# ServiceNow/PipelineRL

Hardware: NVIDIA H100
Metric: rollout_tokens_per_s (higher is better)
Workload: dtype bf16

## Files before the change

include/prl.h:

```cpp
#ifndef PRL_H_
#define PRL_H_

#include <stddef.h>
#include <stdint.h>

#ifdef __cplusplus
extern "C" {
#endif

#define PRL_OK 0
#define PRL_ERR_INVALID (-1)
#define PRL_ERR_CUDA (-2)
#define PRL_ERR_UNSUPPORTED (-3)
#define PRL_ERR_NONFINITE (-4)

typedef void* prl_stream_t;

const char* prl_last_error(void);
int prl_version(void);
uint64_t prl_launch_count(void);
int prl_set_pdl(int32_t on);
int prl_attn_set_fused_combine(int32_t on);


enum { PRL_LOSS_PPO = 0, PRL_LOSS_REINFORCE = 1, PRL_LOSS_GSPO = 2 };

enum {
  PRL_STAT_LOSS = 0, PRL_STAT_MAX_LOSS, PRL_STAT_MIN_LOSS,
  PRL_STAT_REWARD, PRL_STAT_MAX_REWARD, PRL_STAT_MIN_REWARD,
  PRL_STAT_ENTROPY, PRL_STAT_OLD_LOGPROBS, PRL_STAT_NEW_LOGPROBS, PRL_STAT_REF_LOGPROBS,
  PRL_STAT_ADVANTAGE, PRL_STAT_MAX_ADVANTAGE, PRL_STAT_MIN_ADVANTAGE,
  PRL_STAT_KL, PRL_STAT_KL_NEW_OLD, PRL_STAT_MEAN_ABS_LOG_RATIO_NEW_OLD,
  PRL_STAT_MAX_KL, PRL_STAT_MIN_KL,
  PRL_STAT_RATIO_NEW_OLD, PRL_STAT_RATIO_NEW_OLD_SUM, PRL_STAT_RATIO_NEW_OLD_SQUARED_SUM,
  PRL_STAT_RATIO_REF_NEW, PRL_STAT_RATIO_REF_OLD,
  PRL_STAT_CLAMP_LOG_RATIO_REF_NEW_INDICATOR, PRL_STAT_CLAMP_LOG_RATIO_NEW_OLD_INDICATOR,
  PRL_STAT_TOKEN_WEIGHT, PRL_STAT_MAX_TOKEN_WEIGHT, PRL_STAT_MIN_TOKEN_WEIGHT,
  PRL_STAT_KL_COEF, PRL_STAT_ENTROPY_BONUS_COEF,
  PRL_STAT_NUM_OUTPUT_TOKENS_SUM, PRL_STAT_INPUT_SIZE,
  PRL_NUM_STATS
};

typedef struct {
  int32_t policy_loss;
  int32_t use_advantages;
  int32_t relu_log_p_weights;
  int32_t group_normalization;
  int32_t overlong_filtering;
  int32_t use_entropy_loss;
  float epsilon_low, epsilon_high;
  float clamp_log_ratio_ref_new_value;
  float kl_coef;
  float entropy_bonus_coef;
  float batch_size;
} prl_pg_config;

typedef struct {
  int64_t T;
  const float* new_logprobs;
  const float* entropy;
  const int64_t* labels;
  const float* rewards;
  const float* advantages;
  const float* ref_logprobs;
  const float* old_logprobs;
  const float* group_tokens;
  const float* num_labels;
  const float* overflow;
  const int64_t* segment_ids;
  const int64_t* position_ids;
  int32_t n_segments;
  int32_t num_sequences;
  int32_t sentinel;
} prl_pg_batch;

size_t prl_pg_workspace_bytes(int32_t max_segments);

int prl_pg_loss_fwd_bwd(const prl_pg_batch* batch, const prl_pg_config* cfg,
                        float* loss, float* dloss_dlogprob, float* dloss_dentropy,
                        double* stats, int32_t* nonfinite,
                        void* workspace, size_t workspace_bytes, prl_stream_t stream);

int prl_pg_gspo_segment_sums(const prl_pg_batch* batch, const prl_pg_config* cfg, double* seg_sums, prl_stream_t stream);
int prl_pg_loss_fwd_bwd_seg(const prl_pg_batch* batch, const prl_pg_config* cfg, float* loss, float* dloss_dlogprob,
                            float* dloss_dentropy, double* stats, int32_t* nonfinite, void* workspace,
                            size_t workspace_bytes, const double* seg_sums, const double* seg_local_count,
                            prl_stream_t stream);

int prl_logprob_tail_fwd(const float* logits, int64_t T, int64_t V, int64_t row_stride,
                         const int64_t* input_ids, float temperature,
                         float* new_logprobs , float* entropy ,
                         float* lse , prl_stream_t stream);
int prl_logprob_tail_bwd(const float* logits, int64_t T, int64_t V, int64_t row_stride,
                         const int64_t* input_ids, float temperature,
                         const float* lse, const float* entropy,
                         const float* g_logprobs, const float* g_entropy,
                         float* dlogits, int64_t dlogits_stride, prl_stream_t stream);

int prl_logprob_rows_bwd(const float* logits, int64_t n_rows, int64_t V, int64_t row_stride,
                         const int64_t* targets , float temperature, const float* lse,
                         const float* entropy, const float* g_logprobs, const float* g_entropy,
                         float* dlogits, int64_t dlogits_stride, prl_stream_t stream);
int prl_head_dlogits(const void* W_bf16, const void* W_lo_bf16, const void* X_bf16, int64_t M, int64_t V, int64_t K,
                     float temperature, const int64_t* targets, const float* lse, const float* entropy,
                     const float* g_logprobs, const float* g_entropy, void* dz_bf16, int64_t ld_dz, prl_stream_t stream);
// ... 273 lines not shown
```

pipelinerl_b200/_lib.py:

```python
from __future__ import annotations

import ctypes as C
from pathlib import Path

_LIB_PATH = Path(__file__).resolve().parent / "_lib" / "libprl.so"
_lib = None


class PrlError(RuntimeError):
    def __init__(self, code: int, msg: str):
        super().__init__(f"libprl error {code}: {msg}")
        self.code = code


class NonFiniteError(AssertionError):
    """Mirrors the reference's `assert torch.isfinite(...)` (rl/__init__.py:213,263,291,386)."""


class PgConfig(C.Structure):
    _fields_ = [
        ("policy_loss", C.c_int32), ("use_advantages", C.c_int32), ("relu_log_p_weights", C.c_int32),
        ("group_normalization", C.c_int32), ("overlong_filtering", C.c_int32), ("use_entropy_loss", C.c_int32),
        ("epsilon_low", C.c_float), ("epsilon_high", C.c_float), ("clamp_log_ratio_ref_new_value", C.c_float),
        ("kl_coef", C.c_float), ("entropy_bonus_coef", C.c_float), ("batch_size", C.c_float),
# ... 10 lines not shown
        ("n_segments", C.c_int32), ("num_sequences", C.c_int32), ("sentinel", C.c_int32),
    ]


class AdamwArgs(C.Structure):
    _fields_ = [
        ("n", C.c_int64),
        ("master", C.c_void_p), ("exp_avg", C.c_void_p), ("exp_avg_sq", C.c_void_p),
        ("grad", C.c_void_p), ("grad_is_bf16", C.c_int32),
        ("param_bf16", C.c_void_p), ("param_bf16_lo", C.c_void_p),
        ("tensor_offsets", C.c_void_p), ("tensor_no_decay", C.c_void_p), ("n_tensors", C.c_int32),
        ("lr", C.c_double), ("beta1", C.c_double), ("beta2", C.c_double), ("eps", C.c_double),
        ("weight_decay", C.c_double), ("step", C.c_int32), ("max_grad_norm", C.c_float),
        ("grad_scale", C.c_float),
    ]


class AdamwShardArgs(C.Structure):
    _fields_ = [
        ("n", C.c_int64), ("shard_begin", C.c_int64), ("shard_end", C.c_int64),
        ("master", C.c_void_p), ("exp_avg", C.c_void_p), ("exp_avg_sq", C.c_void_p),
        ("grads", C.c_void_p * 8), ("shadows", C.c_void_p * 8), ("norm_tables", C.c_void_p * 8),
        ("n_peers", C.c_int32), ("rank", C.c_int32), ("grad_is_bf16", C.c_int32),
        ("gsum_scratch", C.c_void_p), ("tensor_offsets", C.c_void_p), ("tensor_no_decay", C.c_void_p),
        ("n_tensors", C.c_int32),
        ("lr", C.c_double), ("beta1", C.c_double), ("beta2", C.c_double), ("eps", C.c_double), ("weight_decay", C.c_double),
        ("step", C.c_int32), ("max_grad_norm", C.c_float), ("grad_scale", C.c_float),
    ]


class EngineState(C.Structure):
    _fields_ = [
        ("B", C.c_int32), ("sampled", C.c_void_p), ("sampled_logprobs", C.c_void_p), ("tokens", C.c_void_p),
        ("positions", C.c_void_p), ("seq_lens", C.c_void_p), ("active", C.c_void_p), ("prompt_buf", C.c_void_p),
        ("prompt_stride", C.c_int32), ("prompt_len", C.c_void_p), ("out_ids", C.c_void_p),
        ("out_logprobs", C.c_void_p), ("out_stride", C.c_int32), ("gen_count", C.c_void_p), ("max_new", C.c_void_p),
        ("finished", C.c_void_p), ("eos_id", C.c_int32), ("ignore_eos", C.c_int32), ("ignore_eos_rows", C.c_void_p),
        ("stop_ids", C.c_void_p), ("stop_stride", C.c_int32), ("n_stop", C.c_void_p), ("stop_reason", C.c_void_p),
    ]


class StopStrings(C.Structure):
    _fields_ = [
        ("tok_bytes", C.c_void_p), ("tok_offsets", C.c_void_p), ("tok_special", C.c_void_p), ("vocab", C.c_int32),
        ("stop_str", C.c_void_p), ("stop_str_fail", C.c_void_p), ("stop_str_len", C.c_void_p), ("n_stop_str", C.c_void_p),
        ("max_stop_str", C.c_int32), ("stop_str_stride", C.c_int32), ("stop_str_flags", C.c_void_p),
        ("stop_str_state", C.c_void_p), ("stop_str_match", C.c_void_p), ("min_tokens", C.c_void_p),
    ]


class MbRecord(C.Structure):
    _fields_ = [("n_chunk", C.c_int32), ("n_pack", C.c_int32), ("padding", C.c_int32), ("total_tok", C.c_int32),
                ("total_lp", C.c_int32), ("n_stat_slots", C.c_int32), ("n_rollout_slots", C.c_int32), ("n_groups", C.c_int32),
                ("reward", C.c_void_p), ("stat_slot", C.c_void_p), ("rollout_slot", C.c_void_p), ("group_slot", C.c_void_p),
                ("n_tok_all", C.c_void_p), ("pack_idx", C.c_void_p), ("pack_flags", C.c_void_p), ("tok_off", C.c_void_p),
                ("lp_off", C.c_void_p), ("input_ids", C.c_void_p), ("labels", C.c_void_p), ("logprobs", C.c_void_p),
                ("ref_logprobs", C.c_void_p)]


class MbColumns(C.Structure):
    _fields_ = [(k, C.c_void_p) for k in ("input_ids", "labels", "attention_mask", "position_ids", "segment_ids", "rewards",
                                          "advantages", "ref_logprobs", "old_logprobs", "group_tokens", "num_labels",
                                          "overflow", "seq_boundaries")]


PRL_NUM_STATS = 32
LOSS_IDS = {"ppo": 0, "reinforce": 1, "gspo": 2}
STAT_NAMES = [
    "loss", "max_loss", "min_loss", "reward", "max_reward", "min_reward", "entropy", "old_logprobs",
    "new_logprobs", "ref_logprobs", "advantage", "max_advantage", "min_advantage", "kl", "kl_new_old",
    "mean_abs_log_ratio_new_old", "max_kl", "min_kl", "ratio_new_old", "ratio_new_old_sum",
    "ratio_new_old_squared_sum", "ratio_ref_new", "ratio_ref_old", "clamp_log_ratio_ref_new_indicator",
    "clamp_log_ratio_new_old_indicator", "token_weight", "max_token_weight", "min_token_weight", "kl_coef",
    "entropy_bonus_coef", "num_output_tokens_sum", "input_size",
]
assert len(STAT_NAMES) == PRL_NUM_STATS

_SIGNATURES = {
    "prl_last_error": (C.c_char_p, []),
    "prl_version": (C.c_int, []),
    "prl_launch_count": (C.c_uint64, []),
    "prl_set_pdl": (C.c_int, [C.c_int32]),
    "prl_attn_set_fused_combine": (C.c_int, [C.c_int32]),
    "prl_pg_workspace_bytes": (C.c_size_t, [C.c_int32]),
    "prl_pg_loss_fwd_bwd": (C.c_int, [C.POINTER(PgBatch), C.POINTER(PgConfig), C.c_void_p, C.c_void_p, C.c_void_p,
                                      C.c_void_p, C.c_void_p, C.c_void_p, C.c_size_t, C.c_void_p]),
    "prl_pg_gspo_segment_sums": (C.c_int, [C.POINTER(PgBatch), C.POINTER(PgConfig), C.c_void_p, C.c_void_p]),
    "prl_pg_loss_fwd_bwd_seg": (C.c_int, [C.POINTER(PgBatch), C.POINTER(PgConfig), C.c_void_p, C.c_void_p, C.c_void_p,
                                          C.c_void_p, C.c_void_p, C.c_void_p, C.c_size_t, C.c_void_p, C.c_void_p, C.c_void_p]),
    "prl_logprob_tail_fwd": (C.c_int, [C.c_void_p, C.c_int64, C.c_int64, C.c_int64, C.c_void_p, C.c_float,
                                       C.c_void_p, C.c_void_p, C.c_void_p, C.c_void_p]),
    "prl_logprob_tail_bwd": (C.c_int, [C.c_void_p, C.c_int64, C.c_int64, C.c_int64, C.c_void_p, C.c_float,
                                       C.c_void_p, C.c_void_p, C.c_void_p, C.c_void_p, C.c_void_p, C.c_int64,
                                       C.c_void_p]),
    "prl_gemm_auto_split_k": (C.c_int, [C.c_int64, C.c_int64, C.c_int64]),
    "prl_gemm_set_smem_budget_kb": (C.c_int, [C.c_int32]),
    "prl_gemm_set_tiled_weights": (C.c_int, [C.c_int32]),
    "prl_gemm_tn": (C.c_int, [C.c_void_p, C.c_int64, C.c_void_p, C.c_int64, C.c_int64, C.c_int64, C.c_int64,
                              C.c_void_p, C.c_int64, C.c_int32, C.c_int32, C.c_void_p, C.c_void_p, C.c_int64,
                              C.c_float, C.c_void_p]),
    "prl_rowops_workspace_bytes": (C.c_size_t, [C.c_int64]),
    "prl_rmsnorm_fwd": (C.c_int, [C.c_void_p, C.c_void_p, C.c_int64, C.c_int64, C.c_float, C.c_void_p, C.c_void_p,
                                  C.c_void_p]),
    "prl_rmsnorm_bwd": (C.c_int, [C.c_void_p, C.c_void_p, C.c_void_p, C.c_void_p, C.c_void_p, C.c_int64, C.c_int64,
                                  C.c_void_p, C.c_void_p, C.c_void_p, C.c_size_t, C.c_void_p]),
    "prl_colsum_bf16": (C.c_int, [C.c_void_p, C.c_int64, C.c_int64, C.c_int64, C.c_void_p, C.c_void_p, C.c_size_t,
                                  C.c_void_p]),
    "prl_rope_inplace": (C.c_int, [C.c_void_p, C.c_int64, C.c_int64, C.c_int32, C.c_int32, C.c_void_p, C.c_void_p,
                                   C.c_float, C.c_void_p]),
    "prl_qk_norm_rope_fwd": (C.c_int, [C.c_void_p, C.c_int64, C.c_int64, C.c_int32, C.c_int32, C.c_int32, C.c_void_p,
                                       C.c_void_p, C.c_float, C.c_void_p, C.c_void_p, C.c_void_p, C.c_void_p, C.c_void_p]),
    "prl_qk_norm_rope_bwd": (C.c_int, [C.c_void_p, C.c_int64, C.c_int64, C.c_int32, C.c_int32, C.c_int32, C.c_void_p,
                                       C.c_void_p, C.c_void_p, C.c_void_p, C.c_void_p, C.c_void_p, C.c_void_p, C.c_void_p,
                                       C.c_void_p, C.c_size_t, C.c_void_p]),
    "prl_silu_mul_fwd": (C.c_int, [C.c_void_p, C.c_int64, C.c_int64, C.c_void_p, C.c_void_p]),
    "prl_silu_mul_bwd": (C.c_int, [C.c_void_p, C.c_void_p, C.c_int64, C.c_int64, C.c_void_p, C.c_void_p]),
    "prl_embed_gather": (C.c_int, [C.c_void_p, C.c_void_p, C.c_int64, C.c_int64, C.c_void_p, C.c_void_p]),
    "prl_embed_scatter_add": (C.c_int, [C.c_void_p, C.c_void_p, C.c_void_p, C.c_int64, C.c_int64, C.c_void_p]),
    "prl_gemm_ex": (C.c_int, [C.c_void_p, C.c_int64, C.c_int32, C.c_void_p, C.c_int64, C.c_int32, C.c_int64, C.c_int64,
                              C.c_int64, C.c_void_p, C.c_int64, C.c_int32, C.c_int32, C.c_void_p, C.c_void_p, C.c_int64,
                              C.c_float, C.c_void_p]),
    "prl_transpose_bf16": (C.c_int, [C.c_void_p, C.c_int64, C.c_int64, C.c_int64, C.c_void_p, C.c_int64, C.c_void_p]),
    "prl_gemm_bf16_splitk": (C.c_int, [C.c_void_p, C.c_void_p, C.c_void_p, C.c_int64, C.c_int64, C.c_int64, C.c_int32,
                                       C.c_void_p, C.c_void_p]),
    "prl_head_workspace_bytes": (C.c_size_t, [C.c_int64, C.c_int64]),
    "prl_head_logprob": (C.c_int, [C.c_void_p, C.c_void_p, C.c_void_p, C.c_int64, C.c_int64, C.c_int64, C.c_float,
                                   C.c_void_p, C.c_int32, C.c_uint64, C.c_uint32, C.c_void_p, C.c_void_p, C.c_void_p,
                                   C.c_void_p, C.c_void_p, C.c_void_p, C.c_size_t, C.c_void_p]),
    "prl_embed_rmsnorm": (C.c_int, [C.c_void_p, C.c_void_p, C.c_void_p, C.c_float, C.c_int32, C.c_int32, C.c_int32,
                                    C.c_void_p, C.c_void_p, C.c_void_p]),
    "prl_residual_rmsnorm": (C.c_int, [C.c_void_p, C.c_int32, C.c_int32, C.c_int32, C.c_void_p, C.c_float,
                                       C.c_void_p, C.c_void_p, C.c_void_p, C.c_size_t, C.c_void_p]),
    "prl_qkv_rope_cache": (C.c_int, [C.c_void_p, C.c_int32, C.c_int32, C.c_void_p, C.c_int32, C.c_int32, C.c_int32,
                                     C.c_void_p, C.c_void_p, C.c_int32, C.c_void_p, C.c_void_p, C.c_void_p, C.c_void_p,
                                     C.c_int64, C.c_int32, C.c_int32, C.c_void_p, C.c_size_t, C.c_void_p]),
    "prl_qkv_norm_rope_cache": (C.c_int, [C.c_void_p, C.c_int32, C.c_int32, C.c_void_p, C.c_void_p, C.c_void_p, C.c_float,
                                          C.c_int32, C.c_int32, C.c_int32, C.c_void_p, C.c_void_p, C.c_int32, C.c_void_p,
                                          C.c_void_p, C.c_void_p, C.c_void_p, C.c_int64, C.c_int32, C.c_int32, C.c_void_p,
                                          C.c_size_t, C.c_void_p]),
    "prl_paged_attn_prefill_tc": (C.c_int, [C.c_void_p, C.c_int32, C.c_void_p, C.c_int64, C.c_int32, C.c_int32, C.c_void_p,
                                            C.c_int32, C.c_void_p, C.c_void_p, C.c_void_p, C.c_void_p, C.c_int32,
                                            C.c_int32, C.c_int32, C.c_int32, C.c_int32, C.c_int32, C.c_float,
                                            C.c_void_p, C.c_void_p]),
    "prl_attn_varlen_fwd": (C.c_int, [C.c_void_p, C.c_int64, C.c_int32, C.c_void_p, C.c_void_p, C.c_int32, C.c_int32,
                                      C.c_int32, C.c_int32, C.c_int32, C.c_float, C.c_void_p, C.c_void_p, C.c_void_p]),
    "prl_attn_set_fwd_generation": (C.c_int, [C.c_int32]),
    "prl_attn_set_bwd_generation": (C.c_int, [C.c_int32]),
    "prl_attn_set_prefill_generation": (C.c_int, [C.c_int32]),
    "prl_attn_varlen_bwd_workspace_bytes": (C.c_size_t, [C.c_int32, C.c_int32]),
    "prl_attn_varlen_fwd_kv": (C.c_int, [C.c_void_p, C.c_int64, C.c_int32, C.c_void_p, C.c_int64, C.c_int32, C.c_void_p,
                                         C.c_void_p, C.c_void_p, C.c_void_p, C.c_int32, C.c_int32, C.c_int32, C.c_int32,
                                         C.c_int32, C.c_float, C.c_void_p, C.c_void_p, C.c_void_p]),
    "prl_attn_varlen_bwd_kv": (C.c_int, [C.c_void_p, C.c_int64, C.c_int32, C.c_void_p, C.c_int64, C.c_int32, C.c_void_p,
                                         C.c_void_p, C.c_void_p, C.c_void_p, C.c_int32, C.c_int32, C.c_int32, C.c_int32,
                                         C.c_int32, C.c_int32, C.c_float, C.c_void_p, C.c_void_p, C.c_void_p, C.c_void_p,
                                         C.c_int64, C.c_void_p, C.c_int64, C.c_void_p, C.c_size_t, C.c_void_p]),
    "prl_attn_varlen_bwd": (C.c_int, [C.c_void_p, C.c_int64, C.c_int32, C.c_void_p, C.c_void_p, C.c_int32, C.c_int32,
                                      C.c_int32, C.c_int32, C.c_int32, C.c_float, C.c_void_p, C.c_void_p, C.c_void_p,
                                      C.c_void_p, C.c_int64, C.c_void_p, C.c_size_t, C.c_void_p]),
    "prl_paged_attn_prefill": (C.c_int, [C.c_void_p, C.c_void_p, C.c_int64, C.c_int32, C.c_int32, C.c_void_p,
                                         C.c_int32, C.c_void_p, C.c_void_p, C.c_void_p, C.c_void_p, C.c_int32,
                                         C.c_int32, C.c_int32, C.c_int32, C.c_int32, C.c_int32, C.c_float,
                                         C.c_void_p, C.c_void_p]),
    "prl_silu_mul": (C.c_int, [C.c_void_p, C.c_int32, C.c_int32, C.c_int32, C.c_void_p, C.c_void_p, C.c_size_t,
                               C.c_void_p]),
    "prl_paged_attn_splits": (C.c_int, [C.c_int32, C.c_int32, C.c_int32]),
# ... 97 lines not shown
```

pipelinerl_b200/csrc/decode_ops.cu:

```cuda
#include "prl_common.cuh"
#include <math.h>

namespace prl {
namespace {

__device__ __forceinline__ void l2_prefetch_range(const void* ptr, size_t bytes, size_t tid, size_t nthreads) {
  if (!ptr) return;
  const char* base = static_cast<const char*>(ptr);
  const size_t n_lines = bytes >> 7;
  for (size_t i = tid; i < n_lines; i += nthreads)
    asm volatile("prefetch.global.L2::evict_last [%0];" ::"l"(base + (i << 7)));
}

__device__ __forceinline__ float block_sum(float v, float* s_red) {
  v = warp_sum(v);
  const int lane = threadIdx.x & 31, warp = threadIdx.x >> 5;
  if (lane == 0) s_red[warp] = v;
  __syncthreads();
  float t = 0.f;
  const int nw = (blockDim.x + 31) >> 5;
  for (int i = 0; i < nw; ++i) t += s_red[i];
  __syncthreads();
  return t;
}

__global__ void __launch_bounds__(256) embed_rmsnorm_kernel(const int32_t* __restrict__ tokens,
                                                           const __nv_bfloat16* __restrict__ embed,
                                                           const __nv_bfloat16* __restrict__ gamma, float eps, int H,
                                                           int vocab, float* __restrict__ h,
                                                           __nv_bfloat16* __restrict__ x) {
  pdl_launch_dependents();
  pdl_wait();
  __shared__ float s_red[32];
  const int b = blockIdx.x;
  int tok = tokens[b];
  if (tok < 0 || tok >= vocab) tok = 0;
  const __nv_bfloat16* row = embed + (int64_t)tok * H;
  float ss = 0.f;
  for (int i = threadIdx.x; i < H; i += blockDim.x) {
    const float v = __bfloat162float(row[i]);
    h[(int64_t)b * H + i] = v;
    ss += v * v;
  }
  const float tot = block_sum(ss, s_red);
  const float r = rsqrtf(tot / (float)H + eps);
  for (int i = threadIdx.x; i < H; i += blockDim.x) {
    const float v = __bfloat162float(row[i]);
    x[(int64_t)b * H + i] = __float2bfloat16_rn(v * r * __bfloat162float(gamma[i]));
  }
}

constexpr int kMaxSplitUnroll = 8;
__global__ void __launch_bounds__(1024) residual_rmsnorm_kernel(const float* __restrict__ part, int n_split, int B,
                                                               int H, const __nv_bfloat16* __restrict__ gamma,
                                                               float eps, float* __restrict__ h,
                                                               __nv_bfloat16* __restrict__ x, const void* pf_ptr,
                                                               size_t pf_bytes) {
  pdl_launch_dependents();
  l2_prefetch_range(pf_ptr, pf_bytes, (size_t)blockIdx.x * blockDim.x + threadIdx.x, (size_t)gridDim.x * blockDim.x);
  pdl_wait();
  extern __shared__ float s_row[];
  __shared__ float s_red[32];
  const int b = blockIdx.x;
  const int H4 = H >> 2;
  float4* hrow = reinterpret_cast<float4*>(h + (int64_t)b * H);
  float ss = 0.f;
  float4 keep = make_float4(0.f, 0.f, 0.f, 0.f);
  const bool single = H4 <= (int)blockDim.x;
  for (int i = threadIdx.x; i < H4; i += blockDim.x) {
    float4 v = hrow[i];
    for (int s = 0; s < n_split; s += kMaxSplitUnroll) {
      float4 p[kMaxSplitUnroll];
#pragma unroll
      for (int u = 0; u < kMaxSplitUnroll; ++u)
        if (s + u < n_split) p[u] = reinterpret_cast<const float4*>(part + ((int64_t)(s + u) * B + b) * H)[i];
#pragma unroll
      for (int u = 0; u < kMaxSplitUnroll; ++u)
        if (s + u < n_split) { v.x += p[u].x; v.y += p[u].y; v.z += p[u].z; v.w += p[u].w; }
    }
    hrow[i] = v;
    if (single) keep = v; else reinterpret_cast<float4*>(s_row)[i] = v;
    ss += v.x * v.x + v.y * v.y + v.z * v.z + v.w * v.w;
  }
  const float tot = block_sum(ss, s_red);
  const float r = rsqrtf(tot / (float)H + eps);
  for (int i = threadIdx.x; i < H4; i += blockDim.x) {
    const float4 v = single ? keep : reinterpret_cast<const float4*>(s_row)[i];
    const uint2 gw = reinterpret_cast<const uint2*>(gamma)[i];
    const float g0 = bf16_bits_to_float(gw.x & 0xffffu), g1 = bf16_bits_to_float(gw.x >> 16);
    const float g2 = bf16_bits_to_float(gw.y & 0xffffu), g3 = bf16_bits_to_float(gw.y >> 16);
    const uint32_t o0 = float_to_bf16_bits(v.x * r * g0), o1 = float_to_bf16_bits(v.y * r * g1);
    const uint32_t o2 = float_to_bf16_bits(v.z * r * g2), o3 = float_to_bf16_bits(v.w * r * g3);
    reinterpret_cast<uint2*>(x + (int64_t)b * H)[i] = make_uint2(o0 | (o1 << 16), o2 | (o3 << 16));
  }
}


__device__ __forceinline__ float head_sumsq(float x1, float x2, float* s_ss) {
  float v = warp_sum(__fadd_rn(__fmul_rn(x1, x1), __fmul_rn(x2, x2)));
  const int warp = threadIdx.x >> 5;
  __syncthreads();
  if ((threadIdx.x & 31) == 0) s_ss[warp] = v;
  __syncthreads();
  const int w0 = warp & ~1;
  return __fadd_rn(s_ss[w0], s_ss[w0 + 1]);
}

__device__ __forceinline__ float head_rstd(float ss, float eps) { return rsqrtf(__fmaf_rn(ss, 1.f / 128.f, eps)); }

template <bool kNorm>
__global__ void __launch_bounds__(64) qkv_rope_cache_kernel(const float* __restrict__ part, int n_split, int B,
                                                           const __nv_bfloat16* __restrict__ bias,
                                                           const __nv_bfloat16* __restrict__ q_gamma,
                                                           const __nv_bfloat16* __restrict__ k_gamma, float eps,
                                                           int n_q, int n_kv,
// ... 575 lines not shown
```

pipelinerl_b200/csrc/paged_attn.cu:

```cuda
#include "prl_common.cuh"
#include "tc_ptx.cuh"
#include <math.h>

namespace prl {
namespace {

constexpr int kPage = 64;
constexpr int kD = 128;
constexpr int kStages = 6;
constexpr int kStageBytes = 4 * 8192;
constexpr int kConsumers = 4;
constexpr int kThreads = (kConsumers + 1) * 32;
constexpr int kMaxPagesPerSplit = 1024;

struct AttnParams {
  const __nv_bfloat16* q;
  const int32_t* block_table;
  const int32_t* seq_lens;
  int max_blocks, n_q, n_kv, R;
  int64_t n_pages;
  int layer, n_splits;
  float scale_log2;
  float* o_part;
  float* ml_part;
  unsigned int* tickets;
  __nv_bfloat16* out;
};

__device__ __forceinline__ void ldsm_x4(uint32_t addr, uint32_t& r0, uint32_t& r1, uint32_t& r2, uint32_t& r3) {
  asm volatile("ldmatrix.sync.aligned.m8n8.x4.shared.b16 {%0,%1,%2,%3}, [%4];"
               : "=r"(r0), "=r"(r1), "=r"(r2), "=r"(r3) : "r"(addr));
}
__device__ __forceinline__ void ldsm_x4_t(uint32_t addr, uint32_t& r0, uint32_t& r1, uint32_t& r2, uint32_t& r3) {
  asm volatile("ldmatrix.sync.aligned.m8n8.x4.trans.shared.b16 {%0,%1,%2,%3}, [%4];"
               : "=r"(r0), "=r"(r1), "=r"(r2), "=r"(r3) : "r"(addr));
}
__device__ __forceinline__ void mma_bf16(float (&c)[4], const uint32_t (&a)[4], uint32_t b0, uint32_t b1) {
  asm volatile(
      "mma.sync.aligned.m16n8k16.row.col.f32.bf16.bf16.f32 {%0,%1,%2,%3}, {%4,%5,%6,%7}, {%8,%9}, {%0,%1,%2,%3};"
      : "+f"(c[0]), "+f"(c[1]), "+f"(c[2]), "+f"(c[3])
      : "r"(a[0]), "r"(a[1]), "r"(a[2]), "r"(a[3]), "r"(b0), "r"(b1));
}
__device__ __forceinline__ uint32_t pack_bf16(float lo, float hi) {
  __nv_bfloat162 v = __floats2bfloat162_rn(lo, hi);
  return *reinterpret_cast<uint32_t*>(&v);
}
__device__ __forceinline__ float fast_exp2(float x) {
  float y;
  asm("ex2.approx.ftz.f32 %0, %1;" : "=f"(y) : "f"(x));
  return y;
}

__global__ void __launch_bounds__(kThreads, 1)
paged_attn_decode_kernel(const __grid_constant__ CUtensorMap tm_kv, AttnParams p) {
  extern __shared__ uint8_t smem_raw[];
  const uint32_t base = (ptx::smem_u32(smem_raw) + 1023u) & ~1023u;
  uint8_t* base_ptr = smem_raw + (base - ptx::smem_u32(smem_raw));
  const uint32_t bar_base = base + kStages * kStageBytes;
  auto full_bar = [&](int s) { return bar_base + 8u * (uint32_t)s; };
  auto empty_bar = [&](int s) { return bar_base + 8u * (uint32_t)(kStages + s); };
  int32_t* s_pages = reinterpret_cast<int32_t*>(base_ptr + kStages * kStageBytes + 8 * 2 * kStages);

  const int split = blockIdx.x, kvh = blockIdx.y, b = blockIdx.z;
  const int warp = threadIdx.x >> 5, lane = threadIdx.x & 31;
  pdl_launch_dependents();
  pdl_wait();
  const int seq_len = p.seq_lens[b];
  const int n_pages_b = (seq_len + kPage - 1) / kPage;
  const int per_split = (n_pages_b + p.n_splits - 1) / p.n_splits;
  const int p_begin = split * per_split;
  const int p_end = (p_begin + per_split < n_pages_b) ? p_begin + per_split : n_pages_b;
  const int n_it = p_end > p_begin ? p_end - p_begin : 0;
  const int R = p.R;

  auto finish = [&]() {
    if (p.tickets == nullptr) return;
    __shared__ unsigned int s_ticket;
    __threadfence();
    __syncthreads();
    if (threadIdx.x == 0) s_ticket = atomicAdd(&p.tickets[b * p.n_kv + kvh], 1u);
    __syncthreads();
    if (s_ticket != (unsigned)(p.n_splits - 1)) return;
    __threadfence();
    for (int i = threadIdx.x; i < R * kD; i += kThreads) {
      const int r = i / kD, d = i % kD;
      const int64_t head = (int64_t)b * p.n_q + kvh * R + r;
      float M = -INFINITY;
      for (int sp = 0; sp < p.n_splits; ++sp) M = fmaxf(M, __ldcg(&p.ml_part[(head * p.n_splits + sp) * 2]));
      float L = 0.f, O = 0.f;
      for (int sp = 0; sp < p.n_splits; ++sp) {
        const float ms = __ldcg(&p.ml_part[(head * p.n_splits + sp) * 2]);
        const float f = (ms == -INFINITY) ? 0.f : fast_exp2(ms - M);
        L += __ldcg(&p.ml_part[(head * p.n_splits + sp) * 2 + 1]) * f;
        O += __ldcg(&p.o_part[(head * p.n_splits + sp) * kD + d]) * f;
      }
      p.out[head * kD + d] = __float2bfloat16_rn(L > 0.f ? O / L : 0.f);
    }
    if (threadIdx.x == 0) p.tickets[b * p.n_kv + kvh] = 0u;
  };

  if (n_it == 0) {
    for (int i = threadIdx.x; i < R * kD; i += kThreads) {
      const int r = i / kD, d = i % kD;
      const int64_t head = (int64_t)b * p.n_q + kvh * R + r;
      p.o_part[(head * p.n_splits + split) * kD + d] = 0.f;
      if (d == 0) {
        p.ml_part[(head * p.n_splits + split) * 2 + 0] = -INFINITY;
        p.ml_part[(head * p.n_splits + split) * 2 + 1] = 0.f;
      }
    }
    finish();
    return;
  }

  if (threadIdx.x == 0) {
    for (int s = 0; s < kStages; ++s) {
      ptx::mbar_init(full_bar(s), 1);
      ptx::mbar_init(empty_bar(s), kConsumers);
    }
    ptx::fence_barrier_init();
    ptx::prefetch_tensormap(&tm_kv);
  }
  for (int i = threadIdx.x; i < n_it; i += kThreads)
    s_pages[i] = p.block_table[(int64_t)b * p.max_blocks + p_begin + i];
  __syncthreads();

  float m_run[2] = {-INFINITY, -INFINITY}, l_run[2] = {0.f, 0.f};
  float o[16][4];
#pragma unroll
  for (int i = 0; i < 16; ++i) { o[i][0] = o[i][1] = o[i][2] = o[i][3] = 0.f; }
  const int g = lane >> 2, t = lane & 3;

  if (warp == kConsumers) {
    if (lane == 0) {
      for (int it = 0; it < n_it; ++it) {
        const int s = it % kStages;
        const uint32_t ph = (uint32_t)((it / kStages) & 1);
        ptx::mbar_wait(empty_bar(s), ph ^ 1u);
        ptx::mbar_arrive_expect_tx(full_bar(s), kStageBytes);
        const int page = s_pages[it];
        const int row_k = (int)(((((int64_t)p.layer * 2 + 0) * p.n_pages + page) * p.n_kv + kvh) * kPage);
        const int row_v = (int)(((((int64_t)p.layer * 2 + 1) * p.n_pages + page) * p.n_kv + kvh) * kPage);
        const uint32_t dst = base + (uint32_t)(s * kStageBytes);
        ptx::tma_load_2d(dst, &tm_kv, 0, row_k, full_bar(s), ptx::kEvictFirst);
        ptx::tma_load_2d(dst + 8192, &tm_kv, 64, row_k, full_bar(s), ptx::kEvictFirst);
        ptx::tma_load_2d(dst + 16384, &tm_kv, 0, row_v, full_bar(s), ptx::kEvictFirst);
        ptx::tma_load_2d(dst + 24576, &tm_kv, 64, row_v, full_bar(s), ptx::kEvictFirst);
      }
    }
  } else {
    uint32_t qa[8][4];
    {
      const __nv_bfloat16* qb = p.q + ((int64_t)b * p.n_q + kvh * R) * kD;
#pragma unroll
      for (int ks = 0; ks < 8; ++ks) {
        const int c = ks * 16 + 2 * t;
        qa[ks][0] = (g < R) ? *reinterpret_cast<const uint32_t*>(qb + g * kD + c) : 0u;
        qa[ks][1] = (g + 8 < R) ? *reinterpret_cast<const uint32_t*>(qb + (g + 8) * kD + c) : 0u;
        qa[ks][2] = (g < R) ? *reinterpret_cast<const uint32_t*>(qb + g * kD + c + 8) : 0u;
        qa[ks][3] = (g + 8 < R) ? *reinterpret_cast<const uint32_t*>(qb + (g + 8) * kD + c + 8) : 0u;
      }
    }
    const int mi = lane >> 3, lr = lane & 7;
    for (int it = 0; it < n_it; ++it) {
      const int s = it % kStages;
      const uint32_t ph = (uint32_t)((it / kStages) & 1);
      ptx::mbar_wait(full_bar(s), ph);
      const uint32_t kbase = base + (uint32_t)(s * kStageBytes);
      const uint32_t vbase = kbase + 16384;

      float sc[2][4] = {{0.f, 0.f, 0.f, 0.f}, {0.f, 0.f, 0.f, 0.f}};
      {
        const int row = warp * 16 + (mi >> 1) * 8 + lr;
#pragma unroll
        for (int ks = 0; ks < 8; ++ks) {
          const int chunk = ks * 2 + (mi & 1);
          const uint32_t addr = kbase + (uint32_t)((chunk >> 3) * 8192 + row * 128 + (((chunk & 7) ^ (row & 7)) << 4));
          uint32_t r0, r1, r2, r3;
          ldsm_x4(addr, r0, r1, r2, r3);
          mma_bf16(sc[0], qa[ks], r0, r1);
          mma_bf16(sc[1], qa[ks], r2, r3);
        }
      }
      const int tok0 = (p_begin + it) * kPage + warp * 16;
      const bool tail = tok0 + 16 > seq_len;
#pragma unroll
      for (int nt = 0; nt < 2; ++nt)
#pragma unroll
        for (int e = 0; e < 4; ++e) {
          float v = sc[nt][e] * p.scale_log2;
          if (tail && (tok0 + nt * 8 + 2 * t + (e & 1)) >= seq_len) v = -INFINITY;
          sc[nt][e] = v;
        }
      uint32_t pa[4];
#pragma unroll
      for (int r = 0; r < 2; ++r) {
        float mx = fmaxf(fmaxf(sc[0][2 * r], sc[0][2 * r + 1]), fmaxf(sc[1][2 * r], sc[1][2 * r + 1]));
        mx = fmaxf(mx, __shfl_xor_sync(0xffffffffu, mx, 1));
        mx = fmaxf(mx, __shfl_xor_sync(0xffffffffu, mx, 2));
        const float m_new = fmaxf(m_run[r], mx);
        const float m_use = (m_new == -INFINITY) ? 0.f : m_new;
        const float alpha = fast_exp2(m_run[r] - m_use);
        const float p00 = fast_exp2(sc[0][2 * r] - m_use), p01 = fast_exp2(sc[0][2 * r + 1] - m_use);
        const float p10 = fast_exp2(sc[1][2 * r] - m_use), p11 = fast_exp2(sc[1][2 * r + 1] - m_use);
        l_run[r] = l_run[r] * alpha + (p00 + p01 + p10 + p11);
        m_run[r] = m_new;
#pragma unroll
        for (int i = 0; i < 16; ++i) { o[i][2 * r] *= alpha; o[i][2 * r + 1] *= alpha; }
        pa[r] = pack_bf16(p00, p01);
        pa[2 + r] = pack_bf16(p10, p11);
      }
      {
        const int row = warp * 16 + (mi & 1) * 8 + lr;
#pragma unroll
        for (int dn = 0; dn < 8; ++dn) {
          const int chunk = dn * 2 + (mi >> 1);
          const uint32_t addr = vbase + (uint32_t)((chunk >> 3) * 8192 + row * 128 + (((chunk & 7) ^ (row & 7)) << 4));
          uint32_t r0, r1, r2, r3;
          ldsm_x4_t(addr, r0, r1, r2, r3);
          mma_bf16(o[2 * dn], pa, r0, r1);
          mma_bf16(o[2 * dn + 1], pa, r2, r3);
        }
      }
      __syncwarp();
      if (lane == 0) ptx::mbar_arrive(empty_bar(s));
    }
#pragma unroll
    for (int r = 0; r < 2; ++r) {
      l_run[r] += __shfl_xor_sync(0xffffffffu, l_run[r], 1);
      l_run[r] += __shfl_xor_sync(0xffffffffu, l_run[r], 2);
    }
  }

// ... 167 lines not shown
          const int qpos = pos_first + g + ((e >> 1) ? 8 : 0);
          if (key > qpos) v = -INFINITY;
        }
        sc[nt][e] = v;
      }
#pragma unroll
    for (int r = 0; r < 2; ++r) {
      float mx = -INFINITY;
#pragma unroll
      for (int nt = 0; nt < 8; ++nt) mx = fmaxf(mx, fmaxf(sc[nt][2 * r], sc[nt][2 * r + 1]));
      mx = fmaxf(mx, __shfl_xor_sync(0xffffffffu, mx, 1));
      mx = fmaxf(mx, __shfl_xor_sync(0xffffffffu, mx, 2));
      const float m_new = fmaxf(m_run[r], mx);
      const float m_use = (m_new == -INFINITY) ? 0.f : m_new;
      const float alpha = fast_exp2(m_run[r] - m_use);
      float sum = 0.f;
#pragma unroll
      for (int nt = 0; nt < 8; ++nt) {
        sc[nt][2 * r] = fast_exp2(sc[nt][2 * r] - m_use);
        sc[nt][2 * r + 1] = fast_exp2(sc[nt][2 * r + 1] - m_use);
        sum += sc[nt][2 * r] + sc[nt][2 * r + 1];
      }
      l_run[r] = l_run[r] * alpha + sum;
      m_run[r] = m_new;
#pragma unroll
      for (int i = 0; i < 16; ++i) { o[i][2 * r] *= alpha; o[i][2 * r + 1] *= alpha; }
    }
#pragma unroll
    for (int j = 0; j < 4; ++j) {
      uint32_t pa[4];
      pa[0] = pack_bf16(sc[2 * j][0], sc[2 * j][1]);
      pa[1] = pack_bf16(sc[2 * j][2], sc[2 * j][3]);
      pa[2] = pack_bf16(sc[2 * j + 1][0], sc[2 * j + 1][1]);
      pa[3] = pack_bf16(sc[2 * j + 1][2], sc[2 * j + 1][3]);
      const int row = j * 16 + (mi & 1) * 8 + lr;
#pragma unroll
      for (int dn = 0; dn < 8; ++dn) {
        const int chunk = dn * 2 + (mi >> 1);
        const uint32_t addr = vbase + (uint32_t)((chunk >> 3) * 8192 + row * 128 + (((chunk & 7) ^ (row & 7)) << 4));
        uint32_t r0, r1, r2, r3;
        ldsm_x4_t(addr, r0, r1, r2, r3);
        mma_bf16(o[2 * dn], pa, r0, r1);
        mma_bf16(o[2 * dn + 1], pa, r2, r3);
      }
    }
    __syncwarp();
    if (lane == 0) ptx::mbar_arrive(empty_bar(s));
  }
#pragma unroll
  for (int r = 0; r < 2; ++r) {
    l_run[r] += __shfl_xor_sync(0xffffffffu, l_run[r], 1);
    l_run[r] += __shfl_xor_sync(0xffffffffu, l_run[r], 2);
    const int rowi = g + 8 * r;
    if (rowi < n_valid) {
      const float inv = l_run[r] > 0.f ? 1.f / l_run[r] : 0.f;
      __nv_bfloat16* dst = p.out + ((int64_t)(row0 + rowi) * p.n_q + head) * kD;
#pragma unroll
      for (int i = 0; i < 16; ++i)
        *reinterpret_cast<uint32_t*>(dst + i * 8 + 2 * t) = pack_bf16(o[i][2 * r] * inv, o[i][2 * r + 1] * inv);
    }
  }
}

__global__ void __launch_bounds__(kD) attn_combine_kernel(const float* __restrict__ o_part,
                                                         const float* __restrict__ ml_part, int n_splits,
                                                         __nv_bfloat16* __restrict__ out) {
  const int64_t head = blockIdx.x;
  const int d = threadIdx.x;
  pdl_launch_dependents();
  pdl_wait();
  float M = -INFINITY;
  for (int s = 0; s < n_splits; ++s) M = fmaxf(M, ml_part[(head * n_splits + s) * 2]);
  float L = 0.f, O = 0.f;
  for (int s = 0; s < n_splits; ++s) {
    const float ms = ml_part[(head * n_splits + s) * 2];
    const float f = (ms == -INFINITY) ? 0.f : fast_exp2(ms - M);
    L += ml_part[(head * n_splits + s) * 2 + 1] * f;
    O += o_part[(head * n_splits + s) * kD + d] * f;
  }
  out[head * kD + d] = __float2bfloat16_rn(L > 0.f ? O / L : 0.f);
}

static int g_fused_combine = 0;

}
}

using namespace prl;

extern "C" int prl_attn_set_fused_combine(int32_t on) {
  g_fused_combine = on ? 1 : 0;
  return PRL_OK;
}

extern "C" int prl_paged_attn_splits(int32_t B, int32_t n_kv, int32_t max_seq_len) {
  const int pages = (max_seq_len + kPage - 1) / kPage;
  const int sms = num_sms();
  int splits = 1;
  while (B * n_kv * splits < 2 * sms && pages / (splits * 2) >= 4) splits *= 2;
  while ((pages + splits - 1) / splits > kMaxPagesPerSplit) splits *= 2;
  return splits;
}

extern "C" size_t prl_paged_attn_workspace_bytes(int32_t B, int32_t n_q, int32_t n_splits) {
  return (size_t)B * n_q * n_splits * (kD + 2) * sizeof(float) + (size_t)B * n_q * sizeof(unsigned int);
}

extern "C" int prl_paged_attn_decode(const void* q, const void* kv_cache, int64_t n_pages, int32_t n_layers,
                                     int32_t layer, const int32_t* block_table, int32_t max_blocks,
                                     const int32_t* seq_lens, int32_t B, int32_t n_q, int32_t n_kv, int32_t head_dim,
                                     int32_t page_size, int32_t n_splits, float sm_scale, void* out_bf16,
                                     void* workspace, size_t workspace_bytes, prl_stream_t stream_) {
  PRL_CHECK_ARG(q && kv_cache && block_table && seq_lens && out_bf16 && workspace, "prl_paged_attn_decode: NULL argument");
  PRL_CHECK_ARG(head_dim == kD && page_size == kPage, "prl_paged_attn_decode: head_dim must be 128 and page_size 64");
  PRL_CHECK_ARG(B >= 1 && n_kv >= 1 && n_q % n_kv == 0 && n_q / n_kv <= 16, "prl_paged_attn_decode: need n_q/n_kv <= 16");
  PRL_CHECK_ARG(n_splits >= 1 && layer >= 0 && layer < n_layers, "prl_paged_attn_decode: bad layer/splits");
  PRL_CHECK_ARG((max_blocks + n_splits - 1) / n_splits <= kMaxPagesPerSplit,
                "prl_paged_attn_decode: %d blocks / %d splits exceeds %d pages per CTA", max_blocks, n_splits,
                kMaxPagesPerSplit);
  PRL_CHECK_ARG(workspace_bytes >= prl_paged_attn_workspace_bytes(B, n_q, n_splits), "prl_paged_attn_decode: workspace too small");
  const int64_t total_rows = (int64_t)n_layers * 2 * n_pages * n_kv * kPage;
  PRL_CHECK_ARG(total_rows < (1ll << 31), "prl_paged_attn_decode: KV cache too large for 32-bit TMA row coordinates");
  CUtensorMap tm;
  int rc = make_tmap_2d_bf16(&tm, kv_cache, kD, (uint64_t)total_rows, kD * 2, 64, kPage);
  if (rc) return rc;
  AttnParams p;
  p.q = (const __nv_bfloat16*)q;
  p.block_table = block_table;
  p.seq_lens = seq_lens;
  p.max_blocks = max_blocks; p.n_q = n_q; p.n_kv = n_kv; p.R = n_q / n_kv;
  p.n_pages = n_pages; p.layer = layer; p.n_splits = n_splits;
  p.scale_log2 = sm_scale * 1.4426950408889634f;
  p.o_part = (float*)workspace;
  p.ml_part = p.o_part + (size_t)B * n_q * n_splits * kD;
  p.tickets = g_fused_combine ? reinterpret_cast<unsigned int*>(p.ml_part + (size_t)B * n_q * n_splits * 2) : nullptr;
  p.out = (__nv_bfloat16*)out_bf16;
  const int smem = kStages * kStageBytes + 1024 + 8 * 2 * kStages + 4 * kMaxPagesPerSplit + 16;
  static SmemAttr smem_attr = {};
  PRL_CUDA(ensure_smem(paged_attn_decode_kernel, smem, smem_attr));
  cudaStream_t stream = (cudaStream_t)stream_;
  dim3 grid((unsigned)n_splits, (unsigned)n_kv, (unsigned)B);
  PRL_CUDA(launch_pdl(paged_attn_decode_kernel, grid, dim3(kThreads), (size_t)smem, stream, tm, p));
  PRL_LAUNCH_CHECK();
  if (!g_fused_combine) {
    PRL_CUDA(launch_pdl(attn_combine_kernel, dim3((unsigned)(B * n_q)), dim3(kD), 0, stream, (const float*)p.o_part,
                        (const float*)p.ml_part, (int)n_splits, (__nv_bfloat16*)out_bf16));
    PRL_LAUNCH_CHECK();
  }
  return PRL_OK;
}

extern "C" int prl_paged_attn_prefill(const void* q, const void* kv_cache, int64_t n_pages, int32_t n_layers,
                                      int32_t layer, const int32_t* block_table, int32_t max_blocks,
                                      const int32_t* seq_q_start, const int32_t* seq_q_len, const int32_t* seq_pos0,
                                      const int32_t* seq_slot, int32_t n_seqs, int32_t max_q_len, int32_t n_q,
                                      int32_t n_kv, int32_t head_dim, int32_t page_size, float sm_scale,
                                      void* out_bf16, prl_stream_t stream_) {
  PRL_CHECK_ARG(q && kv_cache && block_table && seq_q_start && seq_q_len && seq_pos0 && seq_slot && out_bf16,
                "prl_paged_attn_prefill: NULL argument");
  PRL_CHECK_ARG(head_dim == kD && page_size == kPage, "prl_paged_attn_prefill: head_dim must be 128 and page_size 64");
  PRL_CHECK_ARG(n_seqs >= 1 && max_q_len >= 1 && n_kv >= 1 && n_q % n_kv == 0 && n_q / n_kv <= kPrefillMaxR,
                "prl_paged_attn_prefill: need n_q/n_kv <= %d", kPrefillMaxR);
  PRL_CHECK_ARG(layer >= 0 && layer < n_layers, "prl_paged_attn_prefill: bad layer");
  const int64_t total_rows = (int64_t)n_layers * 2 * n_pages * n_kv * kPage;
  PRL_CHECK_ARG(total_rows < (1ll << 31), "prl_paged_attn_prefill: KV cache too large for 32-bit TMA row coordinates");
  CUtensorMap tm;
  int rc = make_tmap_2d_bf16(&tm, kv_cache, kD, (uint64_t)total_rows, kD * 2, 64, kPage);
  if (rc) return rc;
  PrefillParams p;
  p.q = (const __nv_bfloat16*)q; p.out = (__nv_bfloat16*)out_bf16;
  p.block_table = block_table; p.seq_q_start = seq_q_start; p.seq_q_len = seq_q_len; p.seq_pos0 = seq_pos0;
  p.seq_slot = seq_slot; p.max_blocks = max_blocks; p.n_q = n_q; p.n_kv = n_kv; p.R = n_q / n_kv;
  p.n_pages = n_pages; p.layer = layer; p.scale_log2 = sm_scale * 1.4426950408889634f;
  const int smem = kStages * kStageBytes + 1024 + 8 * 2 * kStages + 16;
  static SmemAttr smem_attr = {};
  PRL_CUDA(ensure_smem(paged_attn_prefill_kernel, smem, smem_attr));
  dim3 grid((unsigned)((max_q_len + 15) / 16), (unsigned)n_kv, (unsigned)n_seqs);
  PRL_CUDA(launch_pdl(paged_attn_prefill_kernel, grid, dim3((p.R + 1) * 32), (size_t)smem, (cudaStream_t)stream_, tm, p));
  PRL_LAUNCH_CHECK();
  return PRL_OK;
}
```

Measured before the change: 3786.

## Prefetch KV pages before PDL wait and stage fused combine partials in shared memory

Paged attention decode now reads seq_lens and the block table, then issues TMA loads for up to kStages KV pages that are already complete, all before griddepcontrol.wait. This overlaps KV fetch with the tail of the previous kernel. The last page is excluded because it may still be written by the upstream kernel. The fused combine path first copies the split partials into shared memory, so the merge no longer reads global memory repeatedly. The embed kernel now waits on the prior grid before signalling dependents. This relies on the earlier pages and the block table staying unchanged during the prior kernel, which would be a correctness risk if that assumption fails.

New measurement: 3790 (median of 6 runs). No clear change (+0.1%).

```diff
diff --git a/include/prl.h b/include/prl.h
--- a/include/prl.h
+++ b/include/prl.h
@@ -21,6 +21,7 @@
 uint64_t prl_launch_count(void);
 int prl_set_pdl(int32_t on);
 int prl_attn_set_fused_combine(int32_t on);
+int prl_attn_set_prewait(int32_t on);
 
 
 enum { PRL_LOSS_PPO = 0, PRL_LOSS_REINFORCE = 1, PRL_LOSS_GSPO = 2 };
diff --git a/pipelinerl_b200/_lib.py b/pipelinerl_b200/_lib.py
--- a/pipelinerl_b200/_lib.py
+++ b/pipelinerl_b200/_lib.py
@@ -116,6 +116,7 @@
     "prl_launch_count": (C.c_uint64, []),
     "prl_set_pdl": (C.c_int, [C.c_int32]),
     "prl_attn_set_fused_combine": (C.c_int, [C.c_int32]),
+    "prl_attn_set_prewait": (C.c_int, [C.c_int32]),
     "prl_pg_workspace_bytes": (C.c_size_t, [C.c_int32]),
     "prl_pg_loss_fwd_bwd": (C.c_int, [C.POINTER(PgBatch), C.POINTER(PgConfig), C.c_void_p, C.c_void_p, C.c_void_p,
                                       C.c_void_p, C.c_void_p, C.c_void_p, C.c_size_t, C.c_void_p]),
diff --git a/pipelinerl_b200/csrc/decode_ops.cu b/pipelinerl_b200/csrc/decode_ops.cu
--- a/pipelinerl_b200/csrc/decode_ops.cu
+++ b/pipelinerl_b200/csrc/decode_ops.cu
@@ -29,8 +29,8 @@
                                                            const __nv_bfloat16* __restrict__ gamma, float eps, int H,
                                                            int vocab, float* __restrict__ h,
                                                            __nv_bfloat16* __restrict__ x) {
-  pdl_launch_dependents();
-  pdl_wait();
+  pdl_wait();
+  pdl_launch_dependents();
   __shared__ float s_red[32];
   const int b = blockIdx.x;
   int tok = tokens[b];
diff --git a/pipelinerl_b200/csrc/paged_attn.cu b/pipelinerl_b200/csrc/paged_attn.cu
--- a/pipelinerl_b200/csrc/paged_attn.cu
+++ b/pipelinerl_b200/csrc/paged_attn.cu
@@ -20,6 +20,7 @@
   int max_blocks, n_q, n_kv, R;
   int64_t n_pages;
   int layer, n_splits;
+  int prewait;
   float scale_log2;
   float* o_part;
   float* ml_part;
@@ -64,8 +65,8 @@
   const int split = blockIdx.x, kvh = blockIdx.y, b = blockIdx.z;
   const int warp = threadIdx.x >> 5, lane = threadIdx.x & 31;
   pdl_launch_dependents();
-  pdl_wait();
-  const int seq_len = p.seq_lens[b];
+  if (!p.prewait) pdl_wait();
+  const int seq_len = __ldcg(&p.seq_lens[b]);
   const int n_pages_b = (seq_len + kPage - 1) / kPage;
   const int per_split = (n_pages_b + p.n_splits - 1) / p.n_splits;
   const int p_begin = split * per_split;
@@ -82,24 +83,40 @@
     __syncthreads();
     if (s_ticket != (unsigned)(p.n_splits - 1)) return;
     __threadfence();
+    const int64_t head0 = (int64_t)b * p.n_q + kvh * R;
+    const float* op = p.o_part + head0 * p.n_splits * kD;
+    const float* ml = p.ml_part + head0 * p.n_splits * 2;
+    const int n_o = R * p.n_splits * kD, n_ml = R * p.n_splits * 2;
+    const bool staged = (n_o + n_ml) * (int)sizeof(float) <= kStages * kStageBytes;
+    if (staged) {
+      float* s_part = reinterpret_cast<float*>(base_ptr);
+#pragma unroll 4
+      for (int i = threadIdx.x; i < n_o / 4; i += kThreads)
+        reinterpret_cast<float4*>(s_part)[i] = __ldcg(reinterpret_cast<const float4*>(op) + i);
+      for (int i = threadIdx.x; i < n_ml; i += kThreads) s_part[n_o + i] = __ldcg(ml + i);
+      __syncthreads();
+      op = s_part;
+      ml = s_part + n_o;
+    }
+    auto ld = [&](const float* a) { return staged ? *a : __ldcg(a); };
     for (int i = threadIdx.x; i < R * kD; i += kThreads) {
       const int r = i / kD, d = i % kD;
-      const int64_t head = (int64_t)b * p.n_q + kvh * R + r;
       float M = -INFINITY;
-      for (int sp = 0; sp < p.n_splits; ++sp) M = fmaxf(M, __ldcg(&p.ml_part[(head * p.n_splits + sp) * 2]));
+      for (int sp = 0; sp < p.n_splits; ++sp) M = fmaxf(M, ld(&ml[(r * p.n_splits + sp) * 2]));
       float L = 0.f, O = 0.f;
       for (int sp = 0; sp < p.n_splits; ++sp) {
-        const float ms = __ldcg(&p.ml_part[(head * p.n_splits + sp) * 2]);
+        const float ms = ld(&ml[(r * p.n_splits + sp) * 2]);
         const float f = (ms == -INFINITY) ? 0.f : fast_exp2(ms - M);
-        L += __ldcg(&p.ml_part[(head * p.n_splits + sp) * 2 + 1]) * f;
-        O += __ldcg(&p.o_part[(head * p.n_splits + sp) * kD + d]) * f;
-      }
-      p.out[head * kD + d] = __float2bfloat16_rn(L > 0.f ? O / L : 0.f);
+        L += ld(&ml[(r * p.n_splits + sp) * 2 + 1]) * f;
+        O += ld(&op[(r * p.n_splits + sp) * kD + d]) * f;
+      }
+      p.out[(head0 + r) * kD + d] = __float2bfloat16_rn(L > 0.f ? O / L : 0.f);
     }
     if (threadIdx.x == 0) p.tickets[b * p.n_kv + kvh] = 0u;
   };
 
   if (n_it == 0) {
+    pdl_wait();
     for (int i = threadIdx.x; i < R * kD; i += kThreads) {
       const int r = i / kD, d = i % kD;
       const int64_t head = (int64_t)b * p.n_q + kvh * R + r;
@@ -122,7 +139,7 @@
     ptx::prefetch_tensormap(&tm_kv);
   }
   for (int i = threadIdx.x; i < n_it; i += kThreads)
-    s_pages[i] = p.block_table[(int64_t)b * p.max_blocks + p_begin + i];
+    s_pages[i] = __ldcg(&p.block_table[(int64_t)b * p.max_blocks + p_begin + i]);
   __syncthreads();
 
   float m_run[2] = {-INFINITY, -INFINITY}, l_run[2] = {0.f, 0.f};
@@ -132,23 +149,32 @@
   const int g = lane >> 2, t = lane & 3;
 
   if (warp == kConsumers) {
-    if (lane == 0) {
-      for (int it = 0; it < n_it; ++it) {
-        const int s = it % kStages;
-        const uint32_t ph = (uint32_t)((it / kStages) & 1);
-        ptx::mbar_wait(empty_bar(s), ph ^ 1u);
-        ptx::mbar_arrive_expect_tx(full_bar(s), kStageBytes);
-        const int page = s_pages[it];
-        const int row_k = (int)(((((int64_t)p.layer * 2 + 0) * p.n_pages + page) * p.n_kv + kvh) * kPage);
-        const int row_v = (int)(((((int64_t)p.layer * 2 + 1) * p.n_pages + page) * p.n_kv + kvh) * kPage);
-        const uint32_t dst = base + (uint32_t)(s * kStageBytes);
-        ptx::tma_load_2d(dst, &tm_kv, 0, row_k, full_bar(s), ptx::kEvictFirst);
-        ptx::tma_load_2d(dst + 8192, &tm_kv, 64, row_k, full_bar(s), ptx::kEvictFirst);
-        ptx::tma_load_2d(dst + 16384, &tm_kv, 0, row_v, full_bar(s), ptx::kEvictFirst);
-        ptx::tma_load_2d(dst + 24576, &tm_kv, 64, row_v, full_bar(s), ptx::kEvictFirst);
-      }
-    }
+    auto issue = [&](int it) {
+      const int s = it % kStages;
+      const uint32_t ph = (uint32_t)((it / kStages) & 1);
+      ptx::mbar_wait(empty_bar(s), ph ^ 1u);
+      ptx::mbar_arrive_expect_tx(full_bar(s), kStageBytes);
+      const int page = s_pages[it];
+      const int row_k = (int)(((((int64_t)p.layer * 2 + 0) * p.n_pages + page) * p.n_kv + kvh) * kPage);
+      const int row_v = (int)(((((int64_t)p.layer * 2 + 1) * p.n_pages + page) * p.n_kv + kvh) * kPage);
+      const uint32_t dst = base + (uint32_t)(s * kStageBytes);
+      ptx::tma_load_2d(dst, &tm_kv, 0, row_k, full_bar(s), ptx::kEvictFirst);
+      ptx::tma_load_2d(dst + 8192, &tm_kv, 64, row_k, full_bar(s), ptx::kEvictFirst);
+      ptx::tma_load_2d(dst + 16384, &tm_kv, 0, row_v, full_bar(s), ptx::kEvictFirst);
+      ptx::tma_load_2d(dst + 24576, &tm_kv, 64, row_v, full_bar(s), ptx::kEvictFirst);
+    };
+    int n_pre = 0;
+    if (p.prewait) {
+      n_pre = min(min(n_it, kStages), n_pages_b - 1 - p_begin);
+      n_pre = n_pre > 0 ? n_pre : 0;
+    }
+    if (lane == 0)
+      for (int it = 0; it < n_pre; ++it) issue(it);
+    pdl_wait();
+    if (lane == 0)
+      for (int it = n_pre; it < n_it; ++it) issue(it);
   } else {
+    pdl_wait();
     uint32_t qa[8][4];
     {
       const __nv_bfloat16* qb = p.q + ((int64_t)b * p.n_q + kvh * R) * kD;
@@ -482,6 +508,7 @@
 }
 
 static int g_fused_combine = 0;
+static int g_prewait = 1;
 
 }
 }
@@ -490,6 +517,11 @@
 
 extern "C" int prl_attn_set_fused_combine(int32_t on) {
   g_fused_combine = on ? 1 : 0;
+  return PRL_OK;
+}
+
+extern "C" int prl_attn_set_prewait(int32_t on) {
+  g_prewait = on ? 1 : 0;
   return PRL_OK;
 }
 
@@ -530,6 +562,7 @@
   p.seq_lens = seq_lens;
   p.max_blocks = max_blocks; p.n_q = n_q; p.n_kv = n_kv; p.R = n_q / n_kv;
   p.n_pages = n_pages; p.layer = layer; p.n_splits = n_splits;
+  p.prewait = g_prewait;
   p.scale_log2 = sm_scale * 1.4426950408889634f;
   p.o_part = (float*)workspace;
   p.ml_part = p.o_part + (size_t)B * n_q * n_splits * kD;
```
